# timmy139710/HW-Accelerator-Three-Sequence-Alignment

Measured on AMD Instinct MI355X. Metric: GCUPS (10^9 3D-DP cell updates/s), 256^3 cubes, higher is better.
Workload: dtype f16

## Files before the change

hw-accelerator-three-sequence-alignment_amd/csrc/pencil_common.h:

```cpp
#pragma once

#include <algorithm>
#include <cstdlib>
#include <cstdio>
#include <cstring>

#include "pencil_kernel.h"

namespace tsa {

typedef unsigned short u16x2 __attribute__((ext_vector_type(2)));
typedef short s16x2 __attribute__((ext_vector_type(2)));

constexpr size_t LDS_MAX = 160 * 1024;
constexpr int REC_BYTES = 16;
#ifndef TSA_A_B64
#define TSA_A_B64 1
#endif
#ifndef TSA_A_PREFETCH
#define TSA_A_PREFETCH 1
#endif
#ifndef TSA_DMC
#define TSA_DMC 1
#endif
// ... 21 lines not shown
#ifndef TSA_SETPRIO
#define TSA_SETPRIO 1
#endif
#ifndef TSA_IS_STATIC
#define TSA_IS_STATIC 1
#endif
#ifndef TSA_SCHED_FENCE
#define TSA_SCHED_FENCE 1
#endif

struct PencilArgs {
  uint32_t E, O, E2, OE, O2;
  uint32_t f_single, f_pair;
  uint32_t dm, mm;
  uint32_t s3_d1, s3_d0, s3_ne;
  uint32_t h_dm, h_c3;
  uint32_t h_sbc, h_k0, h_kd;
  float dmf;
  int32_t sop;
  int32_t packed;
  int32_t lam;
  uint32_t v_lam, v_cP, v_dO;
  float d0f, d1f;
};


struct LitArgs {
  uint32_t n2E, nOE, n2O;
  uint32_t dmS, mmE, nDOE;
  uint32_t d1S, d0S, neS;
  uint32_t mm3S;
  uint32_t fS[3], fP[2], fM[8];
  int32_t sh, packed;
};
LitArgs lit_args(const KParams &kp);

static inline int32_t pencil_pairs(int32_t max_lc) {
  return max_lc <= 128 ? 1 : max_lc <= 256 ? 2 : max_lc <= 512 ? 4 : 8;
}

__device__ __forceinline__ uint32_t pk_max(uint32_t a, uint32_t b) {
  return __builtin_bit_cast(uint32_t, __builtin_elementwise_max(__builtin_bit_cast(s16x2, a),
                                                                __builtin_bit_cast(s16x2, b)));
}
__device__ __forceinline__ uint32_t pk_sub(uint32_t a, uint32_t b) {
  return __builtin_bit_cast(uint32_t, __builtin_bit_cast(u16x2, a) - __builtin_bit_cast(u16x2, b));
// ... 227 lines not shown
    const h2 eab = H(a[i] & b[i]), eac = H(a[i] & c[i]), DMCi = H(DMC[i]), DMBi = H(DMB[i]);
    const h2 sXY = hfma(eab, DMBi, H(inIxy[i]));
    const h2 sXZ = hfma(eac, DMCi, H(inIxz[i]));
    const h2 sYZ = H(inIyz[i]) + H(SBC[i]);
    h2 sM;
    if constexpr (SOP) sM = hfma(eab, DMBi, hfma(eac, DMCi, H(inM[i]))) + H(K[i]);
    else sM = hfma(eab, H(K[i]), H(inM[i]));
    const h2 sX = H(inIx[i]), sY = H(inIy[i]), sZ = H(inIz[i]);
    const h2 Gx = vmax3(sY, sZ, sYZ), Gy = vmax3(sX, sZ, sXZ), Gz = vmax3(sX, sY, sXY);
    const h2 best = vmax3(Gx, Gy, hmax(sXY, sM));
    const h2 b1 = best - DO;
    const h2 pXY = hmax(Gz, b1), pYZ = hmax(Gx, b1), pXZ = hmax(Gy, b1);
    const h2 qXY = pXY - CP, qYZ = pYZ - CP, qXZ = pXZ - CP;
    oBest[i] = U(best);
    oIxy[i] = U(pXY);
    oIyz[i] = U(pYZ);
    oIxz[i] = U(pXZ);
    nIx[i] = U(vmax3(sX - LAM, qXY, qXZ));
    oIy[i] = U(vmax3(sY - LAM, qXY, qYZ));
    oIz[i] = U(vmax3(sZ - LAM, qYZ, qXZ));
  }
}

template <int M>
__device__ __forceinline__ void zshift(uint32_t (&v)[M], const uint32_t (&src)[M], uint32_t sel,
                                       uint32_t face) {
  const uint32_t r = ror1(src[M - 1]);
#pragma unroll
  for (int i = M - 1; i >= 1; --i) v[i] = src[i - 1];
  v[0] = __builtin_amdgcn_perm(r, face, sel);
}
template <int M>
__device__ __forceinline__ void zfix(uint32_t (&v)[M], const uint32_t (&src)[M], uint32_t sel, uint32_t face) {
#pragma unroll
  for (int i = M - 1; i >= 1; --i) v[i] = src[i];
  v[0] = __builtin_amdgcn_perm(src[0], face, sel);
}
template <int M>
__device__ __forceinline__ void load_a(uint32_t va, uint32_t (&a)[M]) {
#pragma unroll
  for (int i = 0; i < M; ++i)
    a[i] = *(const __attribute__((address_space(3))) uint32_t *)(uintptr_t)(
        va + 4u * (uint32_t)(M - 1 - i));
}
template <int M>
__device__ __forceinline__ void load_a_off(uint32_t va, int off, uint32_t (&a)[M]) {
// ... 14 lines not shown
  const uint64_t lm = 1ull << ls;
  uint32_t m;
  if (hs) asm("v_cndmask_b32_e64 %0, 0, %1, %2 ; hi" : "=v"(m) : "v"(hmHi), "s"(lm));
  else asm("v_cndmask_b32_e64 %0, 0, %1, %2 ; lo" : "=v"(m) : "v"(hmLo), "s"(lm));
  return m;
}
template <int M>
__device__ __forceinline__ void pos_split(int32_t k, int32_t &l, int32_t &i, int32_t &h) {
  const uint32_t u = (uint32_t)k;
  h = (int32_t)(u / (64u * M));
  l = (int32_t)((u / M) & 63u);
  i = (int32_t)(u % M);
}

#define TSA_INLINE_IF_WIDE(call)                 \
  do {                                           \
    if constexpr (M >= 4) {                      \
      [[clang::always_inline]] call;             \
    } else {                                     \
      call;                                      \
    }                                            \
  } while (0)

PencilArgs make_args(const KParams &kp, bool f16, bool vs);

#define TSA_SHAPES(LAUNCH, M_, F16_, SOP_, ...)                                            \
  ((M_) == 1 ? TSA_ARITH(LAUNCH, 1, 8, F16_, SOP_, __VA_ARGS__)                            \
   : (M_) == 2 ? TSA_ARITH(LAUNCH, 2, 8, F16_, SOP_, __VA_ARGS__)                          \
   : (M_) == 4 ? TSA_ARITH(LAUNCH, 4, 8, F16_, SOP_, __VA_ARGS__)                          \
               : TSA_ARITH(LAUNCH, 8, 8, F16_, SOP_, __VA_ARGS__))
#define TSA_ARITH(LAUNCH, MM, NN, F16_, SOP_, ...)                                        \
  ((F16_) ? ((SOP_) ? LAUNCH<MM, NN, true, true>(__VA_ARGS__)                              \
                    : LAUNCH<MM, NN, true, false>(__VA_ARGS__))                            \
          : ((SOP_) ? LAUNCH<MM, NN, false, true>(__VA_ARGS__)                             \
                    : LAUNCH<MM, NN, false, false>(__VA_ARGS__)))

}
```

hw-accelerator-three-sequence-alignment_amd/csrc/pencil_kernel.hip:

```cpp

#include <vector>

#include "pencil_common.h"
#include "h_table.h"
#include "lap_kernel.h"

namespace tsa {


#ifndef TSA_PENCIL_NW
#define TSA_PENCIL_NW 8
#endif
constexpr int PENCIL_NW = TSA_PENCIL_NW;
#ifndef TSA_STORE_SLACK
#define TSA_STORE_SLACK 4
#endif
constexpr int STORE_SLACK = TSA_STORE_SLACK;
constexpr int MAX_LA = 4096, MAX_LB = 4096, MAX_LC = 1024;
__host__ __device__ constexpr int helix_pd(int M) { return M >= 8 ? 2 : M >= 4 ? 4 : 8; }
#ifndef TSA_SKEW
#define TSA_SKEW 2
#endif
__host__ __device__ constexpr int helix_skew(int M) { return M <= 2 ? TSA_SKEW : 1; }
constexpr int RING_EXTRA = 8;
// ... 125 lines not shown
  if (g.M == 2 && !g.two && TSA_EV_STATIC) g.P = (g.P + 3) / 4 * 4;
  g.R = g.P + RING_EXTRA;
  g.ring_bytes_per_triple = (int64_t)g.R * g.M * 64 * REC_BYTES;
  return g;
}
static size_t helix_lds(int M, int NW, int32_t P, int32_t max_lb, bool vs) {
  const size_t a_tab = 4 * ((size_t)P + 128 * M + A_PAD);
  return (size_t)(NW - 1) * 2 * helix_skew(M) * M * 1024 + (size_t)helix_pd(M) * M * 1024 + a_tab +
         4 * (((size_t)max_lb + 3) & ~(size_t)3) + (size_t)M * 512 + (vs && M == 2 && TSA_A_B64 ? a_tab : 0);
}

bool pencil_supported(const tsa_params *p) { return p != nullptr && p->gap_open >= p->gap_extend; }

static bool pencil_shape_ok(int32_t max_la, int32_t max_lb, int32_t max_lc) {
  if (!(max_la >= 1 && max_la <= MAX_LA && max_lb >= 1 && max_lb <= MAX_LB && max_lc >= 1 &&
        max_lc <= MAX_LC))
    return false;
  const PencilGeom g = pencil_geom(max_la, max_lc);
  return helix_lds(g.M, helix_nw(g.M), g.P, max_lb, false) <= LDS_MAX;
}

static bool use_f16(const KParams &kp, const Range &r);
static bool use_vs(const KParams &kp, const Range &r, int32_t max_la, int32_t max_lb, int32_t max_lc);

static double helix_step_us(int M, bool loaded) {
  const double s = M == 1 ? 0.40 : M == 2 ? 0.66 : M == 4 ? 1.2 : 2.4;
  const double alone = M == 1 ? 0.31 : M == 2 ? 0.38 : M == 4 ? 0.7 : 1.4;
  return loaded ? s : alone;
}
static double helix_est(int32_t n, int32_t max_la, int32_t max_lb, int32_t max_lc) {
  const PencilGeom g = pencil_geom(max_la, max_lc);
  const int nw = helix_nw(g.M);
  const int64_t per_cu = std::max<int64_t>(
      1, std::min<int64_t>(LDS_MAX / helix_lds(g.M, nw, g.P, max_lb, g.M == 2), waves_per_cu(g.M) / nw));
  const double T = (double)((max_lb - 1) / nw) * g.P + max_la + nw + max_lc;
  const int64_t units = g.two ? (n + 1) / 2 : n;
  return (double)((units + 256 * per_cu - 1) / (256 * per_cu)) * T *
         helix_step_us(g.M, units > 256);
}

static LapGeom lap_choice(int32_t n, int32_t max_la, int32_t max_lb, int32_t max_lc,
                          LapPolicy lap, bool f16, bool sop, bool need = false) {
  LapGeom none{};
  none.ok = false;
  if (lap == LAP_OFF || max_la > 4096 || max_la + 2 * 8 + 64 * 4 >= 8192) return none;
  char mode[16] = "";
// ... 21 lines not shown
  return pencil_shape_ok(max_la, max_lb, max_lc) &&
         lap_choice(n, max_la, max_lb, max_lc, lap, false, kp.s3_mode == TSA_S3_SOP, true).ok;
}

size_t pencil_workspace_bytes(int32_t n, int32_t max_la, int32_t max_lb, int32_t max_lc,
                              const KParams &kp, const Range &bound, LapPolicy lap, bool checked) {
  if (checked) {
    const LapGeom g = lap_choice(n, max_la, max_lb, max_lc, lap, false, kp.s3_mode == TSA_S3_SOP, true);
    return g.ok ? lap_workspace_bytes(g) : 0;
  }
  if (!pencil_shape_ok(max_la, max_lb, max_lc)) return 0;
  const size_t helix = (size_t)std::min<int32_t>(n, 65535) *
                       (size_t)pencil_geom(max_la, max_lc).ring_bytes_per_triple;
  const LapGeom g = lap_choice(n, max_la, max_lb, max_lc, lap, use_f16(kp, bound),
                               kp.s3_mode == TSA_S3_SOP);
  if (g.ok) return std::max(helix, lap_workspace_bytes(g));
  return helix;
}

bool pencil_shape_supported(int32_t max_la, int32_t max_lb, int32_t max_lc) {
  return pencil_shape_ok(max_la, max_lb, max_lc);
}

template <int M, int NW, bool F16, bool SOP, bool TWO, bool VS>
__global__ __launch_bounds__(64 * NW) void pencil_kernel(const uint8_t *__restrict__ seqs,
                                                         const int64_t *__restrict__ offs,
                                                         int32_t n, int32_t P, int32_t R,
                                                         int32_t lds_a, int32_t lds_b,
                                                         int64_t ring_stride,
                                                         uint8_t *__restrict__ ring_base,
                                                         int32_t *__restrict__ scores,
                                                         PencilArgs pa) {
  extern __shared__ __attribute__((aligned(16))) uint8_t smem[];
  constexpr int PAIR_BYTES = 64 * REC_BYTES;
  constexpr int SLOT_BYTES = M * PAIR_BYTES;
  constexpr int ZT = 128 * M;
  constexpr int PD = helix_pd(M);
  constexpr int HSK = helix_skew(M), HNSL = 2 * HSK;
  uint8_t *xr = smem;
  uint8_t *xr0 = xr + (NW - 1) * HNSL * SLOT_BYTES;
  uint32_t *sA2 = (uint32_t *)(xr0 + PD * SLOT_BYTES);
  uint32_t *sB = (uint32_t *)((uint8_t *)sA2 + lds_a);
  uint32_t *fin = (uint32_t *)((uint8_t *)sB + lds_b);
  uint32_t *sA2s = (uint32_t *)((uint8_t *)fin + M * 512);
  constexpr bool A_B64 = VS && M == 2 && TSA_A_B64;

  const int lane = threadIdx.x & 63;
  const int w = __builtin_amdgcn_readfirstlane(threadIdx.x >> 6);
  static_assert(!TWO || M == 1, "two triples per wave: 64 positions, M = 1");
  static_assert(!VS || (F16 && M <= 2), "V-space: the f16 helix with the four-step loop");
  auto h_bits = [](int32_t v) -> uint32_t {
    const _Float16 h = (_Float16)(float)v;
    return (uint32_t)__builtin_bit_cast(uint16_t, h) * 0x00010001u;
  };
  const uint32_t sel = lane == 0 ? (TWO ? 0x03020100u : 0x05040302u) : 0x07060504u;
  constexpr int KS = TWO ? 64 : 128 * M;
  uint32_t ones = F16 ? 0x08000800u : 0x00010001u;
  asm volatile("" : "+v"(ones));
  constexpr bool SHR = VS && TSA_SHIFTED_REC && !TSA_ABL_ZREC;
  const PencilArgs pv = F16 ? pa : pin_score_consts(pa);
  uint32_t fsv = pa.f_single, fpv = pa.f_pair;
  uint32_t sbcv = pa.h_sbc, kdv = pa.h_kd, k0v = pa.h_k0, one1 = 0x00010001u;
  uint32_t hmLo = TWO ? 0xFFFFFFFFu : 0x0000FFFFu, hmHi = 0xFFFF0000u, zero = 0u;
  if constexpr (!SHR) asm volatile("" : "+v"(fsv), "+v"(fpv), "+v"(sbcv), "+v"(kdv), "+v"(k0v), "+v"(one1));
  if constexpr (!SHR) asm volatile("" : "+v"(hmLo), "+v"(hmHi), "+v"(zero));
  const uint32_t a_lane = (uint32_t)(uintptr_t)(const __attribute__((address_space(3))) void *)sA2 +
                          4u * (uint32_t)(ZT - M * lane - (M - 1));

  uint8_t *rd_wave = w > 0 ? xr + (w - 1) * HNSL * SLOT_BYTES : xr0;
  const lds_u8 *rd_base = to_lds(rd_wave + lane * REC_BYTES);
  lds_u8 *wr_base = to_lds(xr + w * HNSL * SLOT_BYTES + lane * REC_BYTES);
  constexpr bool RP = VS && M == 2 && !TWO && HSK == 2 && TSA_REC_PREV && !SHR && !TSA_ABL_ZREC;
  const lds_u8 *rd_prev = to_lds(rd_wave + ((lane + 63) & 63) * REC_BYTES);
  if constexpr (VS && !SHR && TSA_PIN_BASES) asm volatile("" : "+v"(rd_base), "+v"(wr_base));
  if constexpr (RP && TSA_PIN_BASES) asm volatile("" : "+v"(rd_prev));
  static constexpr HTable H_TABLE = make_h_table();
  constexpr bool HT = VS && M == 2 && !TWO && HSK == 2 && TSA_H_TAB && TSA_EV_STATIC && TSA_HM_TRACK;
  lds_u8 *wrH = to_lds(xr + w * HNSL * SLOT_BYTES + 10);
  const uint32_t own = (uint32_t)lane * REC_BYTES;
  const int32_t nunit = TWO ? (n + 1) / 2 : n;
  for (int unit = blockIdx.x; unit < nunit; unit += gridDim.x) {
    const int tri = TWO ? 2 * unit : unit;
    const int64_t o0 = offs[3 * (int64_t)tri], o1 = offs[3 * (int64_t)tri + 1];
    const int64_t o2 = offs[3 * (int64_t)tri + 2], o3 = offs[3 * (int64_t)tri + 3];
    const int32_t la = (int32_t)(o1 - o0), lb = (int32_t)(o2 - o1), lc = (int32_t)(o3 - o2);
    const bool has1 = TWO && tri + 1 < n;
    const int64_t *of1 = offs + 3 * (int64_t)(has1 ? tri + 1 : tri);
    const int64_t q0 = of1[0], q1 = of1[1], q2 = of1[2];
    const int32_t la1 = TWO ? (int32_t)(q1 - q0) : la, lb1 = TWO ? (int32_t)(q2 - q1) : lb;
    const int32_t lc1 = TWO ? (int32_t)(of1[3] - q2) : lc;
    const int32_t lbm = max(lb, lb1);
    uint8_t *ring = ring_base + (int64_t)blockIdx.x * ring_stride;
    const __amdgpu_buffer_rsrc_t rs_ring = __builtin_amdgcn_make_buffer_rsrc(ring, (short)0, 0x7FFFFFFF, 0x00020000);
    const __amdgpu_buffer_rsrc_t rs_ring63 =
        __builtin_amdgcn_make_buffer_rsrc(ring - 63 * REC_BYTES, (short)0, 0x7FFFFFFF, 0x00020000);

    auto a_entry = [&](int j) -> uint32_t {
      const int x0 = ((j - ZT) % P + P) % P, x1 = TWO ? x0 : ((j - ZT - 64 * M) % P + P) % P;
      const uint32_t c0 = x0 < la ? SYM0 << tsa_sym(seqs, o0 + x0, pa.packed) : 0u;
      const uint32_t c1 = x1 < la1 ? SYM0 << tsa_sym(seqs, (TWO ? q0 : o0) + x1, pa.packed) : 0u;
      return c0 | (c1 << 16);
    };
    for (int j = threadIdx.x; j < P + ZT + A_PAD; j += 64 * NW) {
      sA2[j] = a_entry(j);
      if constexpr (A_B64) sA2s[j] = a_entry(j + 1);
    }
    for (int i = threadIdx.x; i < lbm; i += 64 * NW) {
      if constexpr (TWO)
        sB[i] = (i < lb ? SYM0 << tsa_sym(seqs, o1 + i, pa.packed) : 0u) |
                ((i < lb1 ? SYM0 << tsa_sym(seqs, q1 + i, pa.packed) : 0u) << 16);
      else
        sB[i] = (SYM0 << tsa_sym(seqs, o1 + i, pa.packed)) * 0x00010001u;
    }
    const int32_t lag = P - HSK * (NW - 1);
    constexpr bool FIRSTLAP = VS && TSA_RING_FIRSTLAP;
    const int32_t t_sw = FIRSTLAP ? max(lag - PD, 0) & ~3 : 0;
    if constexpr (FIRSTLAP) {
      const int32_t n16 = (lag - t_sw) * M * 64;
      for (int32_t i = threadIdx.x; i < n16; i += 64 * NW) {
        const int32_t tr = t_sw + i / (M * 64);
        const uint32_t f1 = h_bits(pa.lam * (tr + 1)), f2 = h_bits(pa.lam * (tr + 2));
        ((uint4 *)ring)[(int64_t)(R - lag + tr) * (M * 64) + i % (M * 64)] = make_uint4(f1, f2, f2, f2);
      }
    } else {
      const uint4 face = make_uint4(pa.f_single, pa.f_pair, pa.f_pair, 0u);
      const int64_t n16 = (int64_t)R * M * 64;
      for (int64_t i = threadIdx.x; i < n16; i += 64 * NW) {
        if constexpr (VS) {
          const int32_t tr = (int32_t)((i / (M * 64) + lag) % R);
          const uint32_t f1 = h_bits(pa.lam * (tr + 1)), f2 = h_bits(pa.lam * (tr + 2));
          ((uint4 *)ring)[i] = make_uint4(f1, f2, f2, f2);
        } else {
          ((uint4 *)ring)[i] = face;
        }
      }
    }
    asm volatile("s_waitcnt vmcnt(0) lgkmcnt(0)" ::: "memory");
    __syncthreads();

    uint32_t b[M], c[M], SBC[M], K[M], DMC[M], DMB[M];
    uint32_t oIx[M], shIz[M], svIxy[M], svIyz[M], shIxz[2][M], svM[2][M];
#pragma unroll
    for (int i = 0; i < M; ++i) {
      const int k0 = M * lane + i, k1 = TWO ? k0 : 64 * M + M * lane + i;
      const uint32_t c0 = k0 < lc ? SYM0 << tsa_sym(seqs, o2 + k0, pa.packed) : 0u;
      const uint32_t c1 = k1 < lc1 ? SYM0 << tsa_sym(seqs, (TWO ? q2 : o2) + k1, pa.packed) : 0u;
      c[i] = c0 | (c1 << 16);
      DMC[i] = dm_over_code(pa.dmf, c[i]);
      b[i] = SBC[i] = K[i] = DMB[i] = 0;
      oIx[i] = pa.f_single;
      shIz[i] = pa.f_single;
      shIxz[0][i] = shIxz[1][i] = pa.f_pair;
      svIxy[i] = svIyz[i] = pa.f_pair;
      svM[0][i] = svM[1][i] = 0;
    }
    int32_t xpos0 = (P - ((HSK * w) % P)) % P;
    int32_t lap0 = w == 0 ? 0 : -1;
#if TSA_HM_TRACK
    auto hm_of = [&](int32_t xp) -> uint32_t {
      return xp >= KS ? zero : xp >= 64 * M ? hmHi : hmLo;
    };
    auto ev_of = [&](int32_t xp) -> int32_t { return xp < 64 * M ? 64 * M : xp < KS ? KS : P; };
    uint32_t hmCur = hm_of(xpos0);
    int32_t next_ev = ev_of(xpos0);
#endif
    auto b_of_lap = [&](int32_t lp) -> uint32_t {
      const int32_t r = lp * NW + w;
      return (lp >= 0 && r < lbm) ? sB[r] : 0u;
    };
    uint32_t binj = b_of_lap(lap0);
    uint32_t SBCn[M], Kn[M], DMBn = 0;
    auto row_terms = [&]() {
      if constexpr (F16 && TSA_ROW_NEXT) {
        uint32_t kb0 = k0v, kbd = kdv;
        if constexpr (VS) {
          DMBn = dm_over_code(pa.dmf, binj);
          if constexpr (!SOP) {
            kb0 = dm_over_code(pa.d0f, binj);
            const uint32_t kb1 = dm_over_code(pa.d0f + pa.d1f, binj);
            kbd = (((kb1 & 0xFFFFu) - (kb0 & 0xFFFFu)) & 0xFFFFu) | ((((kb1 >> 16) - (kb0 >> 16)) & 0xFFFFu) << 16);
          }
        }
#pragma unroll
        for (int i = 0; i < M; ++i) {
          const uint32_t e01 = pk_eq1(binj, c[i], one1);
          SBCn[i] = pk_mad(e01, sbcv, 0u);
          Kn[i] = pk_mad(e01, kbd, kb0);
        }
      }
    };
    row_terms();
    const int32_t lap_f = (lb - 1) / NW, w_f = (lb - 1) % NW, k_f = lc - 1;
    const int32_t t_f = lap_f * P + (la - 1) + HSK * w_f + k_f;
    const int32_t w_f1 = (lb1 - 1) % NW, k_f1 = lc1 - 1;
    const int32_t t_f1 = ((lb1 - 1) / NW) * P + (la1 - 1) + HSK * w_f1 + k_f1;
    const int32_t T = (TWO ? max(t_f, t_f1) : t_f) + 1;

    uint32_t Hr[4] = {0u, 0u, 0u, 0u};
    auto hq_at = [&](int32_t s) -> int32_t {
      const int32_t u = s - HSK * w;
      const int32_t lp = u >= 0 ? u / P : -((P - 1 - u) / P);
      return pa.lam * (lp * NW + w + 1 + (u - lp * P));
    };
    auto h_tab = [&](int32_t q) -> uint32_t {
      return H_TABLE.v[min((uint32_t)q, (uint32_t)H_TAB_SAT)];
    };
    auto h_tab4 = [&](auto l1, int32_t q0, uint32_t (&out)[4]) {
      if constexpr (decltype(l1)::value) {
        typedef uint32_t u32x4_a4 __attribute__((ext_vector_type(4), aligned(4)));
        const u32x4_a4 v = *(const u32x4_a4 *)&H_TABLE.v[min((uint32_t)q0, (uint32_t)H_TAB_SAT + 1u)];
        out[0] = v.x, out[1] = v.y, out[2] = v.z, out[3] = v.w;
      } else {
#pragma unroll
        for (int j = 0; j < 4; ++j) out[j] = h_tab(q0 + j * pa.lam);
      }
    };
    int32_t hg = 0;
    uint32_t Hn[4] = {0u, 0u, 0u, 0u}, Hp[4] = {0u, 0u, 0u, 0u};
    if constexpr (VS) {
      if constexpr (HT) {
        Hr[0] = h_tab(hq_at(0));
        Hr[1] = h_tab(hq_at(1));
        Hr[3] = h_tab(hq_at(0) - pa.lam);
        hg = hq_at(1);
        h_tab4(std::false_type{}, hg + pa.lam, Hp);
      } else {
        Hr[0] = h_bits(hq_at(0));
        Hr[1] = h_bits(hq_at(1));
        Hr[3] = U(H(Hr[0]) - H(pa.v_lam));
      }
      if (w == 0) {
#pragma unroll
        for (int i = 0; i < M; ++i) {
          shIz[i] = svIyz[i] = svM[1][i] = Hr[0];
          shIxz[1][i] = Hr[1];
        }
      }
    }
    if constexpr (SHR) {
      if (w == 1 && lane == 0) {
        uint32_t *s0 = (uint32_t *)(xr + 8);
        const uint32_t f1 = h_bits(pa.lam), f2 = h_bits(2 * pa.lam);
        s0[2 * SLOT_BYTES / 4] = s0[2 * SLOT_BYTES / 4 + 1] = f1;
        s0[3 * SLOT_BYTES / 4] = s0[3 * SLOT_BYTES / 4 + 1] = f2;
      }
    }
    int32_t dma_row = 0;
    auto prime = [&](int32_t t0) {
#pragma unroll 1
      for (int s = t0; s < t0 + PD; ++s) {
        const int32_t row = ((s - lag) % R + R) % R;
#pragma unroll
// ... 118 lines not shown
        inIxz[i] = shIxz[PH][i];
        inM[i] = svM[PH][i];
      }
      if (!PRE && !TSA_ABL_INJ && (TSA_HM_TRACK || xpos0 < KS)) {
        int32_t ls, is, hs;
        pos_split<M>(xpos0, ls, is, hs);
#if TSA_HM_TRACK
        uint32_t m1;
        if constexpr (MASK_PAIRS && (PQ & 1)) {
          m1 = m1_pair;
        } else {
          asm("v_cndmask_b32_e64 %0, 0, %1, %2" : "=v"(m1) : "v"(hmCur), "s"(1ull << ls));
          if constexpr (MASK_PAIRS) m1_pair = m1;
        }
#elif TSA_LANE_MASK
        const uint32_t m1 = lane_half_mask(ls, hs, hmLo, hmHi);
#else
        const uint32_t m1 = lane == ls ? (TWO ? 0xFFFFFFFFu : hs ? 0xFFFF0000u : 0x0000FFFFu) : 0u;
#endif
#pragma unroll
        for (int i = 0; i < M; ++i) {
          if (ISC >= 0 ? i == ISC : i == is) {
            if constexpr (VS) {
              if constexpr (HT) {
                inIx[i] = vbfi_s(m1, Hr[PQ & 3], inIx[i]);
                inIxy[i] = vbfi_s(m1, Hr[PQ & 3], inIxy[i]);
                inIxz[i] = vbfi_s(m1, Hr[PQ & 3], inIxz[i]);
                inM[i] = vbfi_s(m1, Hr[(PQ + 3) & 3], inM[i]);
              } else {
                inIx[i] = vbfi(m1, Hr[PQ & 3], inIx[i]);
                inIxy[i] = vbfi(m1, Hr[PQ & 3], inIxy[i]);
                inIxz[i] = vbfi(m1, Hr[PQ & 3], inIxz[i]);
                inM[i] = vbfi(m1, Hr[(PQ + 3) & 3], inM[i]);
              }
            } else {
              inIx[i] = vbfi(m1, fsv, inIx[i]);
              inIxy[i] = vbfi(m1, fpv, inIxy[i]);
              inIxz[i] = vbfi(m1, fpv, inIxz[i]);
              inM[i] = vbfi(m1, zero, inM[i]);
            }
            b[i] = vbfi(m1, binj, b[i]);
            if constexpr (F16) {
#if TSA_ROW_NEXT
              SBC[i] = vbfi(m1, SBCn[i], SBC[i]);
              K[i] = vbfi(m1, Kn[i], K[i]);
              if constexpr (VS) DMB[i] = vbfi(m1, DMBn, DMB[i]);
#else
              const uint32_t e01 = pk_eq1(b[i], c[i], one1);
              SBC[i] = pk_mad(e01, sbcv, 0u);
              K[i] = pk_mad(e01, kdv, k0v);
#endif
            }
          }
        }
      }
#if TSA_PIN_ROW
#pragma unroll
      for (int i = 0; i < M; ++i) asm volatile("" : "+v"(b[i]), "+v"(SBC[i]), "+v"(K[i]), "+v"(DMB[i]));
#endif
      uint32_t oIy[M], oIxy[M], oIyz[M], oBest[M], oIz[M], oIxz[M], nIx[M];
      if constexpr (TSA_SETPRIO) __builtin_amdgcn_s_setprio(0);
      if constexpr (TSA_SCHED_FENCE) __builtin_amdgcn_sched_barrier(0);
      if constexpr (VS)
        cell_messages_vs<M, SOP>(a, b, c, SBC, K, DMC, DMB, pv, inIx, inIy, inIz, inIxy, inIyz, inIxz, inM, nIx,
                                 oIy, oIz, oIxy, oIyz, oIxz, oBest);
      else if constexpr (F16)
        cell_messages_f16<M, SOP>(a, b, c, SBC, K, DMC, ones, pv, inIx, inIy, inIz, inIxy, inIyz, inIxz, inM, nIx,
                             oIy, oIz, oIxy, oIyz, oIxz, oBest);
      else
        cell_messages<M, SOP ? 1 : 0>(a, b, c, ones, pv, inIx, inIy, inIz, inIxy, inIyz, inIxz,
                                      inM, nIx, oIy, oIz, oIxy, oIyz, oIxz, oBest);

      if constexpr (TSA_SCHED_FENCE) __builtin_amdgcn_sched_barrier(0);
      if constexpr (TSA_SETPRIO) __builtin_amdgcn_s_setprio(1);
      if constexpr (TWO) {
        if (t == t_f && w == w_f) fin[lane] = oBest[0];
        if (t == t_f1 && w == w_f1) fin[64 + lane] = oBest[0];
      } else if constexpr (VS) {
        if (t == t_fin) {
#pragma unroll
          for (int i = 0; i < M; ++i) fin[i * 64 + lane] = oBest[i];
        }
      } else if constexpr (FIN) {
        if (w == w_f) {
#pragma unroll
          for (int i = 0; i < M; ++i) fin[i * 64 + lane] = oBest[i];
// ... 98 lines not shown
                if constexpr ((PQ & 3) >= 2) h_tab4(std::bool_constant<L1>{}, hg + pa.lam, Hp);
              } else {
                Hr[PQ & 3] = h_bits(pa.lam * (y - 1));
                Hr[(PQ + 1) & 3] = h_bits(pa.lam * y);
                Hr[(PQ + 2) & 3] = h_bits(pa.lam * (y + 1));
              }
            }
          }
          hmCur = hm_of(xpos0);
          next_ev = ev_of(xpos0);
        }
#else
        static_assert(!VS, "V-space tracks the lap wrap with the half-mask events");
        if (++xpos0 == P) {
          xpos0 = 0;
          binj = b_of_lap(++lap0);
          row_terms();
        }
#endif
      };
      if constexpr (VS) {
        if constexpr (HT) {
          Hr[(PQ + 2) & 3] = Hn[PQ & 3];
        } else {
          Hr[(PQ + 2) & 3] = U(H(Hr[(PQ + 1) & 3]) + H(pa.v_lam));
        }
        advance();
        if constexpr (TSA_ABL_ZOWN) {
          zmove_abl<M>(shIxz[PH], oIxz);
          zmove_abl<M>(shIz, oIz);
        } else {
          zshift<M>(shIxz[PH], oIxz, sel, Hr[(PQ + 2) & 3]);
          zshift<M>(shIz, oIz, sel, Hr[(PQ + 1) & 3]);
        }
        if constexpr (SHR) {
#pragma unroll
          for (int i = 0; i < M; ++i) {
            svIyz[i] = rz[i];
            svM[PH][i] = rw[i];
          }
          const uint32_t face = Hr[(PQ + 2) & 3];
          if (lane == 0) {
            if constexpr (ROLE != 2) {
              lds_u8 *f0 = wr_base + (HSK == 2 ? q : PH) * SLOT_BYTES;
              if constexpr (TWO) {
                lds_w32_at(f0, 8, face);
// ... 151 lines not shown
        TSA_INLINE_IF_WIDE(step(P0, role, t, last));
      }
    };
    constexpr int W0 = (M == 2 && TSA_IS_STATIC) ? 4 : 0, W1 = (M == 2 && TSA_IS_STATIC) ? 8 : 0;
    static_assert(NW % 2 == 0, "the last wave is odd");
    if constexpr (PRE) vs_inject(std::integral_constant<int, 0>{});
    auto run_wave = [&](auto l1) {
      constexpr int LB = decltype(l1)::value ? 16 : 0;
      if (w == 0) TSA_INLINE_IF_WIDE(run(std::integral_constant<int, 0 + W0 + LB>{}));
      else if (w == NW - 1) TSA_INLINE_IF_WIDE(run(std::integral_constant<int, 2 + W1 + LB>{}));
      else if (W0 != 0 && (w & 1)) TSA_INLINE_IF_WIDE(run(std::integral_constant<int, 1 + W1 + LB>{}));
      else TSA_INLINE_IF_WIDE(run(std::integral_constant<int, 1 + W0 + LB>{}));
    };
    if constexpr (HT) {
      if (pa.lam == 1) run_wave(std::true_type{});
      else run_wave(std::false_type{});
    } else {
      TSA_INLINE_IF_WIDE(run_wave(std::false_type{}));
    }
    asm volatile("s_waitcnt vmcnt(0)" ::: "memory");
    __syncthreads();
    if (threadIdx.x == 0) {
      auto decode = [&](uint16_t hb) -> int32_t {
        return F16 ? (int32_t)(float)__builtin_bit_cast(_Float16, hb) : (int32_t)(int16_t)hb;
      };
      const int32_t sh0 = VS ? pa.lam * (la + lb + lc) : 0, sh1 = VS ? pa.lam * (la1 + lb1 + lc1) : 0;
      if constexpr (TWO) {
        scores[tri] = decode((uint16_t)(fin[k_f] & 0xFFFF)) - sh0;
        if (has1) scores[tri + 1] = decode((uint16_t)(fin[64 + k_f1] >> 16)) - sh1;
      } else {
        int32_t l_f, i_f, h_f;
        pos_split<M>(k_f, l_f, i_f, h_f);
        const uint32_t v = fin[i_f * 64 + l_f];
        scores[tri] = decode((uint16_t)(h_f ? (v >> 16) : (v & 0xFFFF))) - sh0;
      }
    }
    __syncthreads();
  }
}

static uint32_t pk16(int32_t v) { return ((uint32_t)(uint16_t)(int16_t)v) * 0x00010001u; }
static uint32_t pkh(double v) {
  const _Float16 h = (_Float16)v;
  uint16_t bits;
  memcpy(&bits, &h, 2);
  return (uint32_t)bits * 0x00010001u;
}

PencilArgs make_args(const KParams &kp, bool f16, bool vs) {
  const int32_t GE = kp.pen[SIXY][SIX], GO = kp.pen[SIXY][SM];
  int32_t fs = -kp.pen[SIX][0], fp = -kp.pen[SIXY][0];
  for (int s = 0; s < 7; ++s) {
    fs = std::max(fs, -kp.pen[SIX][s]);
    fp = std::max(fp, -kp.pen[SIXY][s]);
  }
  PencilArgs a;
  memset(&a, 0, sizeof(a));
  a.sop = kp.s3_mode == TSA_S3_SOP;
  a.packed = kp.packed;
  if (!f16) {
    a.E = pk16(GE);
    a.O = pk16(GO);
    a.E2 = pk16(2 * GE);
    a.OE = pk16(GO + GE);
    a.O2 = pk16(2 * GO);
    a.f_single = pk16(fs);
    a.f_pair = pk16(fp);
    a.dm = pk16(kp.match - kp.mismatch);
    a.mm = pk16(kp.mismatch);
    a.s3_d1 = pk16(kp.s3_eq - kp.s3_ab);
    a.s3_d0 = pk16(kp.s3_ab - kp.s3_ne);
    a.s3_ne = pk16(kp.s3_ne);
// ... 8 lines not shown
  a.f_single = pkh(fs);
  a.f_pair = pkh(fp + mm);
  const int32_t dm = kp.match - mm, d0 = kp.s3_ab - kp.s3_ne, d1 = kp.s3_eq - kp.s3_ab;
  a.h_dm = pkh(dm * 8192.0);
  a.dmf = (float)dm;
  a.h_c3 = pkh((double)kp.s3_ne);
  a.h_sbc = pkh((double)dm);
  const uint32_t k0 = a.sop ? pkh(3.0 * mm) : pkh(d0 * 8192.0);
  const uint32_t k1 = a.sop ? pkh(3.0 * mm + dm) : pkh((d0 + d1) * 8192.0);
  a.h_k0 = k0;
  a.h_kd = (((k1 & 0xFFFF) - (k0 & 0xFFFF)) & 0xFFFF) * 0x00010001u;
  if (vs) {
    a.lam = GE;
    a.v_lam = pkh(GE);
    a.v_cP = pkh(GO + mm + GE);
    a.v_dO = pkh(GO - GE);
    a.d0f = (float)d0;
    a.d1f = (float)d1;
    if (a.sop) {
      const uint32_t k0v = pkh(3.0 * mm + 3.0 * GE), k1v = pkh(3.0 * mm + dm + 3.0 * GE);
      a.h_k0 = k0v;
      a.h_kd = (((k1v & 0xFFFF) - (k0v & 0xFFFF)) & 0xFFFF) * 0x00010001u;
    }
  }
  return a;
}

int64_t pencil_slack(int32_t match, int32_t mismatch, int32_t gap_open, int32_t gap_extend) {
  const int64_t sc = std::max(std::llabs(match), std::llabs(mismatch));
  const int64_t pe = std::max(std::llabs(gap_open), std::llabs(gap_extend));
  return 8 * sc + 4 * pe;
}

static bool arith_override(const char *want) {
  char e[8];
  return override_str("pencil_arith", e, sizeof e) && !strcmp(e, want);
}
static bool use_f16(const KParams &kp, const Range &r) {
  if (arith_override("i16")) return false;
  auto small = [](int64_t v) { return v >= -7 && v <= 7; };
  auto fits = [](int64_t v) { return v >= -2048 && v <= 2048; };
  const int64_t slack = pencil_slack(kp.match, kp.mismatch, kp.pen[SIXY][SM], kp.pen[SIXY][SIX]);
  return r.lo - slack >= -2048 && r.hi + slack <= 2048 &&
         small((int64_t)kp.match - kp.mismatch) && small((int64_t)kp.s3_ab - kp.s3_ne) &&
         small((int64_t)kp.s3_eq - kp.s3_ab) && small((int64_t)kp.s3_eq - kp.s3_ne) &&
         fits(kp.mismatch) && fits(kp.s3_ne) &&
         fits(3LL * kp.mismatch);
}

static bool use_vs(const KParams &kp, const Range &r, int32_t max_la, int32_t max_lb, int32_t max_lc) {
  if (arith_override("i16") || arith_override("f16")) return false;
  const int32_t GE = kp.pen[SIXY][SIX], GO = kp.pen[SIXY][SM];
  if (!use_f16(kp, r) || pencil_pairs(max_lc) > 2 || GE < 1 || GE != -kp.mismatch || GO < GE) return false;
  const PencilGeom g = pencil_geom(max_la, max_lc);
  if (helix_lds(g.M, helix_nw(g.M), g.P, max_lb, true) > LDS_MAX) return false;
  const int64_t slack = pencil_slack(kp.match, kp.mismatch, GO, GE);
  const int64_t hi = r.hi + (int64_t)GE * ((int64_t)max_la + max_lb + max_lc) + slack;
  return r.lo - slack >= -2048 && hi <= 2048 && (int64_t)GO + GE + kp.mismatch <= 2048;
}

static bool lap_vs_ok(const KParams &kp, const Range &r, int32_t max_la, int32_t max_lb, int32_t max_lc) {
  long on = 0;
  if (!override_int("lap_vs", &on) || on == 0) return false;
  if (arith_override("i16") || arith_override("f16")) return false;
  const int32_t GE = kp.pen[SIXY][SIX], GO = kp.pen[SIXY][SM];
  if (!use_f16(kp, r) || GE < 1 || GE != -kp.mismatch || GO < GE) return false;
  const int64_t slack = pencil_slack(kp.match, kp.mismatch, GO, GE);
  const int64_t hi = r.hi + (int64_t)GE * ((int64_t)max_la + max_lb + max_lc) + slack;
  return r.lo - slack >= -2048 && hi <= 2048 && (int64_t)GO + GE + kp.mismatch <= 2048;
}

template <int M, int NW, bool F16, bool SOP>
static int launch_m(const uint8_t *d_seqs, const int64_t *d_offsets, int32_t n,
                    int32_t max_lb, const PencilGeom &g, int32_t *d_scores, void *d_ws,
                    const PencilArgs &pa, hipStream_t stream) {
  constexpr bool VSOK = F16 && M <= 2;
  const bool vs = VSOK && pa.lam != 0;
  const int32_t lds_a = 4 * (g.P + 128 * M + A_PAD), lds_b = 4 * ((max_lb + 3) & ~3);
  const size_t lds = helix_lds(M, NW, g.P, max_lb, vs);
  const bool two = M == 1 && g.two;
  auto kfn = vs ? (two ? pencil_kernel<M, NW, F16, SOP, M == 1, VSOK> : pencil_kernel<M, NW, F16, SOP, false, VSOK>)
                : (two ? pencil_kernel<M, NW, F16, SOP, M == 1, false> : pencil_kernel<M, NW, F16, SOP, false, false>);
  if (lds > LDS_MAX) return TSA_EINVAL;
  const int32_t units = two ? (n + 1) / 2 : n;
  const int grid = units < 65535 ? units : 65535;
  return launch_with_lds((const void *)kfn, lds, [&] {
           hipLaunchKernelGGL(kfn, dim3(grid), dim3(64 * NW), lds, stream, d_seqs, d_offsets, n, g.P, g.R, lds_a,
                              lds_b, g.ring_bytes_per_triple, (uint8_t *)d_ws, d_scores, pa);
         }) == hipSuccess
             ? TSA_OK
             : TSA_EDEVICE;
}

void pencil_describe(int32_t n, int32_t max_la, int32_t max_lb, int32_t max_lc, const KParams &kp,
                     const Range &bound, LapPolicy lap, char *buf, size_t len, bool checked) {
  const bool f16 = checked ? false : use_f16(kp, bound);
  const char *arith = f16 ? "f16" : "i16";
  const char *s3 = kp.s3_mode == TSA_S3_SOP ? "sop" : "rtl";
  const LapGeom lg = lap_choice(n, max_la, max_lb, max_lc, lap, f16, kp.s3_mode == TSA_S3_SOP, checked);
  if (lg.ok) {
    if (f16 && lap_vs_ok(kp, bound, max_la, max_lb, max_lc)) arith = "f16v";
    char chunk[32] = "";
    if (lg.chunk > 0) snprintf(chunk, sizeof chunk, " chunk=%d", lg.chunk);
    snprintf(buf, len, "pencil lap %s %s M=%d NW=%d laps=%d tiles=%d waves=%lld wpc=%d%s%s est=%.0fus", arith, s3,
             lg.M, lg.NW, lg.G, lg.GZ, (long long)lg.waves, lg.per_cu, chunk, checked ? " checked" : "", lg.est_us);
    return;
  }
  const PencilGeom g = pencil_geom(max_la, max_lc);
  if (use_vs(kp, bound, max_la, max_lb, max_lc)) arith = "f16v";
  snprintf(buf, len, "pencil helix %s %s M=%d NW=%d P=%d%s est=%.0fus", arith, s3, g.M, helix_nw(g.M), g.P,
           g.two ? " two" : "", helix_est(n, max_la, max_lb, max_lc));
}

int pencil_launch_batch(const uint8_t *d_seqs, const int64_t *d_offsets, int32_t n,
                        int32_t max_la, int32_t max_lb, int32_t max_lc, const KParams &kp,
                        const Range &bound, int32_t *d_scores, void *d_ws, size_t ws_bytes,
                        hipStream_t stream, LapPolicy lap, int32_t **d_err,
                        const CheckLimits *chk) {
  if (d_err) *d_err = nullptr;
  if (n <= 0) return TSA_OK;
  if (!pencil_shape_ok(max_la, max_lb, max_lc)) return TSA_EINVAL;
  const bool f16 = chk ? false : use_f16(kp, bound);
  const bool sop = kp.s3_mode == TSA_S3_SOP;
  const LapGeom lg = lap_choice(n, max_la, max_lb, max_lc, lap, f16, sop, chk != nullptr);
  if (lg.ok) {
    if (ws_bytes < lap_workspace_bytes(lg)) return TSA_ENOMEM;
    const bool lvs = f16 && lap_vs_ok(kp, bound, max_la, max_lb, max_lc);
    return lap_launch(lg, f16, sop, d_seqs, d_offsets, n, d_scores, d_ws, make_args(kp, f16, lvs), stream,
                      d_err, chk);
  }
  const PencilArgs pa = make_args(kp, f16, !chk && use_vs(kp, bound, max_la, max_lb, max_lc));
  if (chk) return TSA_ERANGE;
  const PencilGeom g = pencil_geom(max_la, max_lc);
  const int32_t grid = n < 65535 ? n : 65535;
  if (ws_bytes < (size_t)grid * (size_t)g.ring_bytes_per_triple) return TSA_ENOMEM;
  if (PENCIL_NW != 8 && g.M == 2 && f16 && !sop)
    return launch_m<2, PENCIL_NW, true, false>(d_seqs, d_offsets, n, max_lb, g, d_scores, d_ws, pa, stream);
  return TSA_SHAPES(launch_m, g.M, f16, sop, d_seqs, d_offsets, n, max_lb, g,
                    d_scores, d_ws, pa, stream);
}

LapGeom pencil_split_geom(int32_t la, int32_t lb, int32_t lc, const KParams &kp, const Range &bound,
                          int np) {
  LapGeom g{};
  g.ok = false;
  if (np < 1 || !pencil_shape_ok(la, lb, lc)) return g;
  const bool f16 = use_f16(kp, bound), sop = kp.s3_mode == TSA_S3_SOP;
  g = lap_choice(1, la, lb, lc, LAP_RESIDENT, f16, sop, true);
  if (!g.ok || g.G < np) {
    g.ok = false;
    return g;
  }
  return lap_geom(1, la, lb, lc, g.M, g.NW, true, f16, sop);
}
// ... 11 lines not shown
```

Baseline: 1959.

## Add integer-pattern V-space helix variant using biased scaled scores in f16 bit space

Adds a VI mode for the M=2 V-space helix kernel. Scores are stored as biased integers scaled by 8, kept in the range where positive f16 bit patterns sort the same way as integers. That lets the cell update use plain packed integer add, sub and mad while still using f16 max for comparisons. The host computes a bias from the score range bounds and turns the path on by default when everything fits, otherwise it falls back to the float V-space path. This is meant to replace f16 arithmetic with cheaper or more exact integer ops. The risk is carries crossing between the two 16-bit lanes if the range analysis is wrong, plus extra sign-fixup work when rows are set up.

```diff
diff --git a/hw-accelerator-three-sequence-alignment_amd/csrc/pencil_common.h b/hw-accelerator-three-sequence-alignment_amd/csrc/pencil_common.h
--- a/hw-accelerator-three-sequence-alignment_amd/csrc/pencil_common.h
+++ b/hw-accelerator-three-sequence-alignment_amd/csrc/pencil_common.h
@@ -67,6 +67,10 @@
   int32_t lam;
   uint32_t v_lam, v_cP, v_dO;
   float d0f, d1f;
+  int32_t bias;
+  uint32_t i_bias;
+  uint32_t i_lam, i_cP, i_dO;
+  int32_t dm8, d0_8, d1_8;
 };
 
 
@@ -340,6 +344,55 @@
   }
 }
 
+__device__ __forceinline__ uint32_t imax(uint32_t a, uint32_t b) { return U(hmax(H(a), H(b))); }
+__device__ __forceinline__ uint32_t imax3(uint32_t a, uint32_t b, uint32_t c) {
+  return U(vmax3(H(a), H(b), H(c)));
+}
+__device__ __forceinline__ uint32_t w8_over_code(int32_t w8, uint32_t codes) {
+  uint32_t r = 0;
+#pragma unroll
+  for (int h = 0; h < 2; ++h) {
+    const int32_t c = (int32_t)((codes >> (16 * h)) & 0xFFFFu);
+    if (c != 0) r |= ((uint32_t)(w8 / c) & 0xFFFFu) << (16 * h);
+  }
+  return r;
+}
+__device__ __forceinline__ uint32_t pk_signed(uint32_t v) { return v - ((v & 0x8000u) << 1); }
+template <int M, bool SOP>
+__device__ __forceinline__ void cell_messages_vi(
+    const uint32_t (&a)[M], const uint32_t (&b)[M], const uint32_t (&c)[M],
+    const uint32_t (&SBC)[M], const uint32_t (&K)[M], const uint32_t (&DMC)[M], const uint32_t (&DMB)[M],
+    const PencilArgs &pa,
+    const uint32_t (&inIx)[M], const uint32_t (&inIy)[M], const uint32_t (&inIz)[M],
+    const uint32_t (&inIxy)[M], const uint32_t (&inIyz)[M], const uint32_t (&inIxz)[M],
+    const uint32_t (&inM)[M], uint32_t (&nIx)[M], uint32_t (&oIy)[M], uint32_t (&oIz)[M],
+    uint32_t (&oIxy)[M], uint32_t (&oIyz)[M], uint32_t (&oIxz)[M], uint32_t (&oBest)[M]) {
+  const uint32_t LAM = pa.i_lam, CP = pa.i_cP, DO = pa.i_dO;
+#pragma unroll
+  for (int i = 0; i < M; ++i) {
+    const uint32_t eab = a[i] & b[i], eac = a[i] & c[i];
+    const uint32_t sXY = pk_mad(eab, DMB[i], inIxy[i]);
+    const uint32_t sXZ = pk_mad(eac, DMC[i], inIxz[i]);
+    const uint32_t sYZ = inIyz[i] + SBC[i];
+    uint32_t sM;
+    if constexpr (SOP) sM = pk_mad(eab, DMB[i], pk_mad(eac, DMC[i], inM[i])) + K[i];
+    else sM = pk_mad(eab, K[i], inM[i]);
+    const uint32_t sX = inIx[i], sY = inIy[i], sZ = inIz[i];
+    const uint32_t Gx = imax3(sY, sZ, sYZ), Gy = imax3(sX, sZ, sXZ), Gz = imax3(sX, sY, sXY);
+    const uint32_t best = imax3(Gx, Gy, imax(sXY, sM));
+    const uint32_t b1 = best - DO;
+    const uint32_t pXY = imax(Gz, b1), pYZ = imax(Gx, b1), pXZ = imax(Gy, b1);
+    const uint32_t qXY = pXY - CP, qYZ = pYZ - CP, qXZ = pXZ - CP;
+    oBest[i] = best;
+    oIxy[i] = pXY;
+    oIyz[i] = pYZ;
+    oIxz[i] = pXZ;
+    nIx[i] = imax3(sX - LAM, qXY, qXZ);
+    oIy[i] = imax3(sY - LAM, qXY, qYZ);
+    oIz[i] = imax3(sZ - LAM, qYZ, qXZ);
+  }
+}
+
 template <int M>
 __device__ __forceinline__ void zshift(uint32_t (&v)[M], const uint32_t (&src)[M], uint32_t sel,
                                        uint32_t face) {
@@ -400,7 +453,7 @@
     }                                            \
   } while (0)
 
-PencilArgs make_args(const KParams &kp, bool f16, bool vs);
+PencilArgs make_args(const KParams &kp, bool f16, bool vs, int32_t vi_bias = 0);
 
 #define TSA_SHAPES(LAUNCH, M_, F16_, SOP_, ...)                                            \
   ((M_) == 1 ? TSA_ARITH(LAUNCH, 1, 8, F16_, SOP_, __VA_ARGS__)                            \
diff --git a/hw-accelerator-three-sequence-alignment_amd/csrc/pencil_kernel.hip b/hw-accelerator-three-sequence-alignment_amd/csrc/pencil_kernel.hip
--- a/hw-accelerator-three-sequence-alignment_amd/csrc/pencil_kernel.hip
+++ b/hw-accelerator-three-sequence-alignment_amd/csrc/pencil_kernel.hip
@@ -171,6 +171,7 @@
 
 static bool use_f16(const KParams &kp, const Range &r);
 static bool use_vs(const KParams &kp, const Range &r, int32_t max_la, int32_t max_lb, int32_t max_lc);
+static int32_t use_vi(const KParams &kp, const Range &r, int32_t max_la, int32_t max_lb, int32_t max_lc);
 
 static double helix_step_us(int M, bool loaded) {
   const double s = M == 1 ? 0.40 : M == 2 ? 0.66 : M == 4 ? 1.2 : 2.4;
@@ -238,7 +239,7 @@
   return pencil_shape_ok(max_la, max_lb, max_lc);
 }
 
-template <int M, int NW, bool F16, bool SOP, bool TWO, bool VS>
+template <int M, int NW, bool F16, bool SOP, bool TWO, bool VS, bool VI = false>
 __global__ __launch_bounds__(64 * NW) void pencil_kernel(const uint8_t *__restrict__ seqs,
                                                          const int64_t *__restrict__ offs,
                                                          int32_t n, int32_t P, int32_t R,
@@ -265,9 +266,17 @@
   const int w = __builtin_amdgcn_readfirstlane(threadIdx.x >> 6);
   static_assert(!TWO || M == 1, "two triples per wave: 64 positions, M = 1");
   static_assert(!VS || (F16 && M <= 2), "V-space: the f16 helix with the four-step loop");
-  auto h_bits = [](int32_t v) -> uint32_t {
+  static_assert(!VI || (VS && M == 2 && !TWO && helix_skew(M) == 2 && !TSA_H_TAB && !TSA_SHIFTED_REC && !TSA_PREINJ),
+                "integer patterns: the V-space M = 2 helix at skew 2");
+  constexpr uint32_t SYMC = VI ? 1u : SYM0;
+  auto h_bits = [&](int32_t v) -> uint32_t {
+    if constexpr (VI) return (uint32_t)(pa.bias + 8 * v) * 0x00010001u;
     const _Float16 h = (_Float16)(float)v;
     return (uint32_t)__builtin_bit_cast(uint16_t, h) * 0x00010001u;
+  };
+  auto w_over_code = [&](float wf, int32_t w8, uint32_t codes) -> uint32_t {
+    if constexpr (VI) return w8_over_code(w8, codes);
+    else return dm_over_code(wf, codes);
   };
   const uint32_t sel = lane == 0 ? (TWO ? 0x03020100u : 0x05040302u) : 0x07060504u;
   constexpr int KS = TWO ? 64 : 128 * M;
@@ -313,8 +322,8 @@
 
     auto a_entry = [&](int j) -> uint32_t {
       const int x0 = ((j - ZT) % P + P) % P, x1 = TWO ? x0 : ((j - ZT - 64 * M) % P + P) % P;
-      const uint32_t c0 = x0 < la ? SYM0 << tsa_sym(seqs, o0 + x0, pa.packed) : 0u;
-      const uint32_t c1 = x1 < la1 ? SYM0 << tsa_sym(seqs, (TWO ? q0 : o0) + x1, pa.packed) : 0u;
+      const uint32_t c0 = x0 < la ? SYMC << tsa_sym(seqs, o0 + x0, pa.packed) : 0u;
+      const uint32_t c1 = x1 < la1 ? SYMC << tsa_sym(seqs, (TWO ? q0 : o0) + x1, pa.packed) : 0u;
       return c0 | (c1 << 16);
     };
     for (int j = threadIdx.x; j < P + ZT + A_PAD; j += 64 * NW) {
@@ -323,10 +332,10 @@
     }
     for (int i = threadIdx.x; i < lbm; i += 64 * NW) {
       if constexpr (TWO)
-        sB[i] = (i < lb ? SYM0 << tsa_sym(seqs, o1 + i, pa.packed) : 0u) |
-                ((i < lb1 ? SYM0 << tsa_sym(seqs, q1 + i, pa.packed) : 0u) << 16);
+        sB[i] = (i < lb ? SYMC << tsa_sym(seqs, o1 + i, pa.packed) : 0u) |
+                ((i < lb1 ? SYMC << tsa_sym(seqs, q1 + i, pa.packed) : 0u) << 16);
       else
-        sB[i] = (SYM0 << tsa_sym(seqs, o1 + i, pa.packed)) * 0x00010001u;
+        sB[i] = (SYMC << tsa_sym(seqs, o1 + i, pa.packed)) * 0x00010001u;
     }
     const int32_t lag = P - HSK * (NW - 1);
     constexpr bool FIRSTLAP = VS && TSA_RING_FIRSTLAP;
@@ -359,16 +368,16 @@
 #pragma unroll
     for (int i = 0; i < M; ++i) {
       const int k0 = M * lane + i, k1 = TWO ? k0 : 64 * M + M * lane + i;
-      const uint32_t c0 = k0 < lc ? SYM0 << tsa_sym(seqs, o2 + k0, pa.packed) : 0u;
-      const uint32_t c1 = k1 < lc1 ? SYM0 << tsa_sym(seqs, (TWO ? q2 : o2) + k1, pa.packed) : 0u;
+      const uint32_t c0 = k0 < lc ? SYMC << tsa_sym(seqs, o2 + k0, pa.packed) : 0u;
+      const uint32_t c1 = k1 < lc1 ? SYMC << tsa_sym(seqs, (TWO ? q2 : o2) + k1, pa.packed) : 0u;
       c[i] = c0 | (c1 << 16);
-      DMC[i] = dm_over_code(pa.dmf, c[i]);
+      DMC[i] = w_over_code(pa.dmf, pa.dm8, c[i]);
       b[i] = SBC[i] = K[i] = DMB[i] = 0;
       oIx[i] = pa.f_single;
       shIz[i] = pa.f_single;
       shIxz[0][i] = shIxz[1][i] = pa.f_pair;
       svIxy[i] = svIyz[i] = pa.f_pair;
-      svM[0][i] = svM[1][i] = 0;
+      svM[0][i] = svM[1][i] = VI ? pa.i_bias : 0u;
     }
     int32_t xpos0 = (P - ((HSK * w) % P)) % P;
     int32_t lap0 = w == 0 ? 0 : -1;
@@ -390,10 +399,10 @@
       if constexpr (F16 && TSA_ROW_NEXT) {
         uint32_t kb0 = k0v, kbd = kdv;
         if constexpr (VS) {
-          DMBn = dm_over_code(pa.dmf, binj);
+          DMBn = w_over_code(pa.dmf, pa.dm8, binj);
           if constexpr (!SOP) {
-            kb0 = dm_over_code(pa.d0f, binj);
-            const uint32_t kb1 = dm_over_code(pa.d0f + pa.d1f, binj);
+            kb0 = w_over_code(pa.d0f, pa.d0_8, binj);
+            const uint32_t kb1 = w_over_code(pa.d0f + pa.d1f, pa.d0_8 + pa.d1_8, binj);
             kbd = (((kb1 & 0xFFFFu) - (kb0 & 0xFFFFu)) & 0xFFFFu) | ((((kb1 >> 16) - (kb0 >> 16)) & 0xFFFFu) << 16);
           }
         }
@@ -402,6 +411,10 @@
           const uint32_t e01 = pk_eq1(binj, c[i], one1);
           SBCn[i] = pk_mad(e01, sbcv, 0u);
           Kn[i] = pk_mad(e01, kbd, kb0);
+          if constexpr (VI) {
+            SBCn[i] = pk_signed(SBCn[i]);
+            if constexpr (SOP) Kn[i] = pk_signed(Kn[i]);
+          }
         }
       }
     };
@@ -443,7 +456,8 @@
       } else {
         Hr[0] = h_bits(hq_at(0));
         Hr[1] = h_bits(hq_at(1));
-        Hr[3] = U(H(Hr[0]) - H(pa.v_lam));
+        if constexpr (VI) Hr[3] = Hr[0] - pa.i_lam;
+        else Hr[3] = U(H(Hr[0]) - H(pa.v_lam));
       }
       if (w == 0) {
 #pragma unroll
@@ -608,7 +622,7 @@
         for (int i = 0; i < M; ++i) {
           if (ISC >= 0 ? i == ISC : i == is) {
             if constexpr (VS) {
-              if constexpr (HT) {
+              if constexpr (HT || VI) {
                 inIx[i] = vbfi_s(m1, Hr[PQ & 3], inIx[i]);
                 inIxy[i] = vbfi_s(m1, Hr[PQ & 3], inIxy[i]);
                 inIxz[i] = vbfi_s(m1, Hr[PQ & 3], inIxz[i]);
@@ -647,7 +661,10 @@
       uint32_t oIy[M], oIxy[M], oIyz[M], oBest[M], oIz[M], oIxz[M], nIx[M];
       if constexpr (TSA_SETPRIO) __builtin_amdgcn_s_setprio(0);
       if constexpr (TSA_SCHED_FENCE) __builtin_amdgcn_sched_barrier(0);
-      if constexpr (VS)
+      if constexpr (VI)
+        cell_messages_vi<M, SOP>(a, b, c, SBC, K, DMC, DMB, pv, inIx, inIy, inIz, inIxy, inIyz, inIxz, inM, nIx,
+                                 oIy, oIz, oIxy, oIyz, oIxz, oBest);
+      else if constexpr (VS)
         cell_messages_vs<M, SOP>(a, b, c, SBC, K, DMC, DMB, pv, inIx, inIy, inIz, inIxy, inIyz, inIxz, inM, nIx,
                                  oIy, oIz, oIxy, oIyz, oIxz, oBest);
       else if constexpr (F16)
@@ -792,6 +809,8 @@
       if constexpr (VS) {
         if constexpr (HT) {
           Hr[(PQ + 2) & 3] = Hn[PQ & 3];
+        } else if constexpr (VI) {
+          Hr[(PQ + 2) & 3] = Hr[(PQ + 1) & 3] + pa.i_lam;
         } else {
           Hr[(PQ + 2) & 3] = U(H(Hr[(PQ + 1) & 3]) + H(pa.v_lam));
         }
@@ -989,6 +1008,7 @@
     __syncthreads();
     if (threadIdx.x == 0) {
       auto decode = [&](uint16_t hb) -> int32_t {
+        if constexpr (VI) return ((int32_t)hb - pa.bias) / 8;
         return F16 ? (int32_t)(float)__builtin_bit_cast(_Float16, hb) : (int32_t)(int16_t)hb;
       };
       const int32_t sh0 = VS ? pa.lam * (la + lb + lc) : 0, sh1 = VS ? pa.lam * (la1 + lb1 + lc1) : 0;
@@ -1014,7 +1034,7 @@
   return (uint32_t)bits * 0x00010001u;
 }
 
-PencilArgs make_args(const KParams &kp, bool f16, bool vs) {
+PencilArgs make_args(const KParams &kp, bool f16, bool vs, int32_t vi_bias) {
   const int32_t GE = kp.pen[SIXY][SIX], GO = kp.pen[SIXY][SM];
   int32_t fs = -kp.pen[SIX][0], fp = -kp.pen[SIXY][0];
   for (int s = 0; s < 7; ++s) {
@@ -1069,6 +1089,20 @@
       a.h_k0 = k0v;
       a.h_kd = (((k1v & 0xFFFF) - (k0v & 0xFFFF)) & 0xFFFF) * 0x00010001u;
     }
+    if (vi_bias != 0) {
+      a.bias = vi_bias;
+      a.i_bias = (uint32_t)vi_bias * 0x00010001u;
+      a.i_lam = (uint32_t)(8 * GE) * 0x00010001u;
+      a.i_cP = (uint32_t)(8 * (GO + mm + GE)) * 0x00010001u;
+      a.i_dO = (uint32_t)(8 * (GO - GE)) * 0x00010001u;
+      a.dm8 = 8 * dm;
+      a.d0_8 = 8 * d0;
+      a.d1_8 = 8 * d1;
+      a.f_single = a.f_pair = a.i_bias;
+      a.h_sbc = pk16(8 * dm);
+      a.h_k0 = pk16(8 * (3 * mm + 3 * GE));
+      a.h_kd = pk16(8 * dm);
+    }
   }
   return a;
 }
@@ -1104,6 +1138,29 @@
   const int64_t slack = pencil_slack(kp.match, kp.mismatch, GO, GE);
   const int64_t hi = r.hi + (int64_t)GE * ((int64_t)max_la + max_lb + max_lc) + slack;
   return r.lo - slack >= -2048 && hi <= 2048 && (int64_t)GO + GE + kp.mismatch <= 2048;
+}
+
+#ifndef TSA_VI_DEFAULT
+#define TSA_VI_DEFAULT 1
+#endif
+constexpr int32_t VI_LO = 0x0400, VI_HI = 0x7BFF;
+constexpr bool VI_BUILT = TSA_REC_PREV && !TSA_H_TAB && !TSA_SHIFTED_REC && !TSA_PREINJ && TSA_SKEW == 2 &&
+                          PENCIL_NW == 8;
+static int32_t use_vi(const KParams &kp, const Range &r, int32_t max_la, int32_t max_lb, int32_t max_lc) {
+  if (arith_override("f16vf") || !use_vs(kp, r, max_la, max_lb, max_lc)) return 0;
+  if (!TSA_VI_DEFAULT && !arith_override("f16vi")) return 0;
+  const PencilGeom g = pencil_geom(max_la, max_lc);
+  if (!VI_BUILT || g.M != 2 || g.two) return 0;
+  const int32_t GE = kp.pen[SIXY][SIX], GO = kp.pen[SIXY][SM];
+  const int64_t e_la = g.P, e_lb = (int64_t)max_lb + 2 * helix_nw(g.M), e_lc = 128 * g.M;
+  const int64_t mn = std::min<int64_t>(max_la, std::min(max_lb, max_lc)), e_mn = std::min(e_la, std::min(e_lb, e_lc));
+  const int64_t q = (int64_t)max_la + max_lb + max_lc, e_q = e_la + e_lb + e_lc;
+  const int64_t lo = -((-std::min<int64_t>(r.lo, 0) * e_mn + mn - 1) / mn);
+  const int64_t hi = ((std::max<int64_t>(r.hi, 0) + 1) * e_q + q - 1) / q;
+  const int64_t slack = pencil_slack(kp.match, kp.mismatch, GO, GE);
+  const int64_t v_lo = lo - slack, v_hi = hi + (int64_t)GE * e_q + slack;
+  if (8 * (v_hi - v_lo) > VI_HI - VI_LO) return 0;
+  return (int32_t)(VI_LO - 8 * v_lo);
 }
 
 static bool lap_vs_ok(const KParams &kp, const Range &r, int32_t max_la, int32_t max_lb, int32_t max_lc) {
@@ -1128,6 +1185,9 @@
   const bool two = M == 1 && g.two;
   auto kfn = vs ? (two ? pencil_kernel<M, NW, F16, SOP, M == 1, VSOK> : pencil_kernel<M, NW, F16, SOP, false, VSOK>)
                 : (two ? pencil_kernel<M, NW, F16, SOP, M == 1, false> : pencil_kernel<M, NW, F16, SOP, false, false>);
+  if constexpr (VSOK && M == 2 && VI_BUILT) {
+    if (vs && pa.bias != 0) kfn = pencil_kernel<M, NW, F16, SOP, false, VSOK, true>;
+  }
   if (lds > LDS_MAX) return TSA_EINVAL;
   const int32_t units = two ? (n + 1) / 2 : n;
   const int grid = units < 65535 ? units : 65535;
@@ -1155,8 +1215,9 @@
   }
   const PencilGeom g = pencil_geom(max_la, max_lc);
   if (use_vs(kp, bound, max_la, max_lb, max_lc)) arith = "f16v";
+  const bool vi = !checked && use_vi(kp, bound, max_la, max_lb, max_lc) != 0;
   snprintf(buf, len, "pencil helix %s %s M=%d NW=%d P=%d%s est=%.0fus", arith, s3, g.M, helix_nw(g.M), g.P,
-           g.two ? " two" : "", helix_est(n, max_la, max_lb, max_lc));
+           g.two ? " two" : vi ? " int" : "", helix_est(n, max_la, max_lb, max_lc));
 }
 
 int pencil_launch_batch(const uint8_t *d_seqs, const int64_t *d_offsets, int32_t n,
@@ -1170,13 +1231,15 @@
   const bool f16 = chk ? false : use_f16(kp, bound);
   const bool sop = kp.s3_mode == TSA_S3_SOP;
   const LapGeom lg = lap_choice(n, max_la, max_lb, max_lc, lap, f16, sop, chk != nullptr);
+  const int32_t vi_bias = chk ? 0 : use_vi(kp, bound, max_la, max_lb, max_lc);
+  if (arith_override("f16vi") && (lg.ok || vi_bias == 0)) return TSA_EINVAL;
   if (lg.ok) {
     if (ws_bytes < lap_workspace_bytes(lg)) return TSA_ENOMEM;
     const bool lvs = f16 && lap_vs_ok(kp, bound, max_la, max_lb, max_lc);
     return lap_launch(lg, f16, sop, d_seqs, d_offsets, n, d_scores, d_ws, make_args(kp, f16, lvs), stream,
                       d_err, chk);
   }
-  const PencilArgs pa = make_args(kp, f16, !chk && use_vs(kp, bound, max_la, max_lb, max_lc));
+  const PencilArgs pa = make_args(kp, f16, !chk && use_vs(kp, bound, max_la, max_lb, max_lc), vi_bias);
   if (chk) return TSA_ERANGE;
   const PencilGeom g = pencil_geom(max_la, max_lc);
   const int32_t grid = n < 65535 ? n : 65535;
```

Result: faster. 2016, median of 6 (+2.9%).
